# UtkuKaradeniz/scrabble-gan

Measured on AMD Instinct MI355X. Metric: train-step images/sec @ 32×160 bs128, 1/2/4/8 GPU; % of HBM/MFMA roofline, higher is better.
Workload: dtype f32

## Files before the change

scrabble_gan_amd/csrc/conv_bf16v2.hip:

```cpp
#include "sg_conv2.h"
#include <stdlib.h>
#include <type_traits>

typedef float f32x16 __attribute__((ext_vector_type(16)));
typedef __bf16 bf16x8 __attribute__((ext_vector_type(8)));
typedef short s16x8 __attribute__((ext_vector_type(8)));
__device__ __attribute__((aligned(256))) unsigned int sg2_zero_page[64];

__device__ __forceinline__ int sg2_xcd_remap(int orig, int nwg) {
  const int q = nwg >> 3, r = nwg & 7, xcd = orig & 7;
  const int base = xcd < r ? xcd * (q + 1) : r * (q + 1) + (xcd - r) * q;
  return base + (orig >> 3);
}

__global__ __launch_bounds__(256) void k_cvt_bf16(const float* __restrict__ x, u16* __restrict__ out, long n8, int relu,
                                                  const float* __restrict__ rowscale, long rowlen) {
  for (long e = (long)blockIdx.x * blockDim.x + threadIdx.x; e < n8; e += (long)gridDim.x * blockDim.x) {
    float4 v0 = reinterpret_cast<const float4*>(x)[2 * e], v1 = reinterpret_cast<const float4*>(x)[2 * e + 1];
    if (rowscale) {
      const float s = rowscale[(8 * e) / rowlen];
      v0.x *= s; v0.y *= s; v0.z *= s; v0.w *= s; v1.x *= s; v1.y *= s; v1.z *= s; v1.w *= s;
    }
    if (relu) {
      v0.x = fmaxf(v0.x, 0.f); v0.y = fmaxf(v0.y, 0.f); v0.z = fmaxf(v0.z, 0.f); v0.w = fmaxf(v0.w, 0.f);
      v1.x = fmaxf(v1.x, 0.f); v1.y = fmaxf(v1.y, 0.f); v1.z = fmaxf(v1.z, 0.f); v1.w = fmaxf(v1.w, 0.f);
    }
    bf16x8 h;
    h[0] = (__bf16)v0.x; h[1] = (__bf16)v0.y; h[2] = (__bf16)v0.z; h[3] = (__bf16)v0.w;
    h[4] = (__bf16)v1.x; h[5] = (__bf16)v1.y; h[6] = (__bf16)v1.z; h[7] = (__bf16)v1.w;
    reinterpret_cast<bf16x8*>(out)[e] = h;
  }
}

extern "C" int sg_cvt_bf16(const float* x, void* out, long n, int relu, const float* rowscale, long rowlen, void* stream) {
  if (!x || !out || n < 0 || (n & 7) || (rowscale && (rowlen <= 0 || (rowlen & 7)))) return SG_ERR_ARG;
  if (n == 0) return SG_OK;
  SG_KERNEL(k_cvt_bf16, dim3(sg_grid_for(n / 8, 256)), dim3(256), 0, (hipStream_t)stream, x, (u16*)out, n / 8, relu, rowscale, rowlen);
  return sg_launch_status();
}

__global__ __launch_bounds__(256) void k_cvt_bf16_bias(const float* __restrict__ x, u16* __restrict__ out, u16* __restrict__ out_plain, long M,
                                                       int C, const float* __restrict__ rowscale, long rows_per_sample,
                                                       float* __restrict__ dbias, int rows_per_block) {
  __shared__ float red[256 * 8];
  const int c8 = C >> 3;
  int CL = 256;
  while (CL > c8) CL >>= 1;
  const int RL = 256 / CL;
  const int cl = threadIdx.x % CL, rl = threadIdx.x / CL;
  const long m0 = (long)blockIdx.x * rows_per_block;
  const long m1 = m0 + rows_per_block < M ? m0 + rows_per_block : M;
  for (int cg0 = 0; cg0 < c8; cg0 += CL) {
    const int cg = cg0 + cl;
    float s[8] = {0.f, 0.f, 0.f, 0.f, 0.f, 0.f, 0.f, 0.f};
    if (cg < c8) {
      for (long m = m0 + rl; m < m1; m += RL) {
        const float4* src = reinterpret_cast<const float4*>(x + m * C + 8 * cg);
        float4 v0 = src[0], v1 = src[1];
        if (out_plain) {
          bf16x8 hp;
          hp[0] = (__bf16)v0.x; hp[1] = (__bf16)v0.y; hp[2] = (__bf16)v0.z; hp[3] = (__bf16)v0.w;
          hp[4] = (__bf16)v1.x; hp[5] = (__bf16)v1.y; hp[6] = (__bf16)v1.z; hp[7] = (__bf16)v1.w;
          *reinterpret_cast<bf16x8*>(out_plain + m * C + 8 * cg) = hp;
        }
        if (rowscale) {
          const float f = rowscale[m / rows_per_sample];
          v0.x *= f; v0.y *= f; v0.z *= f; v0.w *= f; v1.x *= f; v1.y *= f; v1.z *= f; v1.w *= f;
        }
        bf16x8 hh;
        hh[0] = (__bf16)v0.x; hh[1] = (__bf16)v0.y; hh[2] = (__bf16)v0.z; hh[3] = (__bf16)v0.w;
        hh[4] = (__bf16)v1.x; hh[5] = (__bf16)v1.y; hh[6] = (__bf16)v1.z; hh[7] = (__bf16)v1.w;
        *reinterpret_cast<bf16x8*>(out + m * C + 8 * cg) = hh;
        s[0] += v0.x; s[1] += v0.y; s[2] += v0.z; s[3] += v0.w; s[4] += v1.x; s[5] += v1.y; s[6] += v1.z; s[7] += v1.w;
      }
    }
    if (RL > 1) {
#pragma unroll
      for (int j = 0; j < 8; ++j) red[j * 256 + threadIdx.x] = s[j];
      __syncthreads();
      for (int st = RL >> 1; st > 0; st >>= 1) {
        if (rl < st) {
#pragma unroll
          for (int j = 0; j < 8; ++j) red[j * 256 + threadIdx.x] += red[j * 256 + threadIdx.x + st * CL];
        }
        __syncthreads();
      }
#pragma unroll
      for (int j = 0; j < 8; ++j) s[j] = red[j * 256 + threadIdx.x];
      __syncthreads();
    }
    if (rl == 0 && cg < c8) {
#pragma unroll
      for (int j = 0; j < 8; ++j) atomicAdd(dbias + 8 * cg + j, s[j]);
    }
  }
}

extern "C" int sg_cvt_bf16_bias(const float* x, void* out, void* out_plain, long M, int C, const float* rowscale, long rows_per_sample,
                                float* dbias, void* stream) {
  if (!x || !out || !dbias || M < 0 || C <= 0 || (C & 7) || (rowscale && rows_per_sample <= 0)) return SG_ERR_ARG;
  if (M == 0) return SG_OK;
  long r = (M + 1023) / 1024;
  if (sg_deterministic()) r = M;
  const int rpb = (int)(r < 32 ? 32 : r);
  SG_KERNEL(k_cvt_bf16_bias, dim3((unsigned)((M + rpb - 1) / rpb)), dim3(256), 0, (hipStream_t)stream, x, (u16*)out, (u16*)out_plain, M, C,
                     rowscale, rows_per_sample, dbias, rpb);
  return sg_launch_status();
}

constexpr int SG2_BM = 256, SG2_BK = 64;
constexpr int SG2_TILE = SG2_BM * SG2_BK * 2;
constexpr int SG2_LDS = 4 * SG2_TILE;

template <int BN, int ES, bool RELU, int BMT = 256, int NWO = 0>
__global__ __launch_bounds__((NWO ? NWO : (BMT == 256 ? 8 : 4)) * 64, 2) void sg_igemm_bf16v2_kernel(const SgIgemm2Args p) {
  extern __shared__ __attribute__((aligned(1024))) unsigned char smem[];
  constexpr int BM = BMT, BK = 128 / ES;
  constexpr int NW = NWO ? NWO : (BM == 256 ? 8 : 4);
  constexpr int ATILE = BM * 128;
  constexpr int WN = BN / 64, WM = NW / WN;
  constexpr int TM = BM / WM / 32, TN = 2;
  constexpr int BQ = BN / (8 * NW);
  constexpr int AQ = BM / (8 * NW);
  static_assert(BM == 256 || (BM == 128 && (BN == 128 || (BN == 64 && ES == 4))), "tile configurations");
  static_assert(NWO == 0 || (NWO == 8 && BM == 128 && ES == 4), "eight waves: the fp32 128 x 128 tile only");
  constexpr int BTILE = BN * 128;
  const int tid = threadIdx.x;
  const int lane = tid & 63;
  const int wave = __builtin_amdgcn_readfirstlane(tid >> 6);
  const int wm = wave / WN, wn = wave % WN;

  const int M = p.Bn * p.Hg * p.Wg;
  const int HW = p.Hg * p.Wg;
  const int n_tiles = p.N / BN;
  int wg, split, nsplit;
  int bid = (int)blockIdx.x;
  if constexpr (ES == 4 && BMT == 128) bid += p.block0;
  if (bid < p.full_tiles) {
    wg = sg2_xcd_remap(bid, p.full_tiles);
    split = 0;
    nsplit = 1;
  } else {
    const int tail_tiles = p.n_tiles_total - p.full_tiles;
    const int u = sg2_xcd_remap(bid - p.full_tiles, tail_tiles * p.tail_split);
    nsplit = p.tail_split;
    split = u / tail_tiles;
    wg = p.full_tiles + (u - split * tail_tiles);
  }
  const int m0 = (wg / n_tiles) * BM;
  const int n0 = (wg % n_tiles) * BN;
  const int grp = p.group_rows ? m0 / p.group_rows : 0;
  const int grp_row0 = grp * p.group_rows;
  const int kchunks = p.Ca / BK;
  const int KT_all = p.ntaps * kchunks;
  const int kt_begin = (int)(((long)KT_all * split) / nsplit);
  const int KT = (int)(((long)KT_all * (split + 1)) / nsplit) - kt_begin;

  const int lrow = lane >> 3, lslot = lane & 7;
  const unsigned char* zero = reinterpret_cast<const unsigned char*>(sg2_zero_page) + 16 * lslot;
  unsigned a_off[4], a_msk[4], b_off[4];
#pragma unroll
  for (int i = 0; i < 4; ++i) {
    const int r = (NW * i + wave) * 8 + lrow;
    const int chunk = lslot ^ ((r >> 1) & 7);
    const int m = m0 + r;
    const bool ok = m < M;
// ... 1389 lines not shown
```

scrabble_gan_amd/csrc/conv_winograd.hip:

```cpp
#include "sg_conv2.h"
#include "wino_f43.h"
#include <stdlib.h>

#define WINO_F 16

static inline long wino_tp(long T) { return (T + 127) / 128 * 128; }


__global__ __launch_bounds__(256) void k_wino_filter(const float* __restrict__ in, float* __restrict__ U, long NK, int flip) {
  for (long e = (long)blockIdx.x * 256 + threadIdx.x; e < NK; e += (long)gridDim.x * 256) {
    float g[3][3];
#pragma unroll
    for (int a = 0; a < 3; ++a)
#pragma unroll
      for (int b = 0; b < 3; ++b) g[a][b] = in[(size_t)((flip ? 2 - a : a) * 3 + (flip ? 2 - b : b)) * NK + e];
    float h[4][3];
#pragma unroll
    for (int b = 0; b < 3; ++b) {
      h[0][b] = g[0][b];
      h[1][b] = 0.5f * (g[0][b] + g[1][b] + g[2][b]);
      h[2][b] = 0.5f * (g[0][b] - g[1][b] + g[2][b]);
      h[3][b] = g[2][b];
    }
#pragma unroll
// ... 438 lines not shown
  return (long)sizeof(float) * wino_planes(tile) * wino_tp(wino_tiles(B, H, W, tile)) * ((long)Cin + Cout);
}

extern "C" int sg_wino_filter(const float* w_nk, float* u, int N, int K, int flip, int tile, void* stream) {
  if (!w_nk || !u || N <= 0 || K <= 0 || (tile != 2 && tile != 4)) return SG_ERR_ARG;
  const long NK = (long)N * K;
  if (tile == 2) SG_KERNEL(k_wino_filter, dim3(sg_grid_for(NK, 256)), dim3(256), 0, (hipStream_t)stream, w_nk, u, NK, flip);
  else SG_KERNEL(k_w43_filter, dim3(sg_grid_for(NK, 256)), dim3(256), 0, (hipStream_t)stream, w_nk, u, NK, flip);
  return sg_launch_status();
}

static int wino_input_impl(const float* x, float* V, int B, int H, int W, int C, int relu, int tile, int ups, void* stream);
extern "C" int sg_wino_input(const float* x, float* V, int B, int H, int W, int C, int relu, int tile, void* stream) {
  return wino_input_impl(x, V, B, H, W, C, relu, tile, 0, stream);
}
extern "C" int sg_wino_input_ups(const float* x_half, float* V, int B, int H, int W, int C, int tile, void* stream) {
  if (tile != 4) return SG_ERR_UNSUPPORTED;
  return wino_input_impl(x_half, V, B, H, W, C, 0, tile, 1, stream);
}
static int wino_input_impl(const float* x, float* V, int B, int H, int W, int C, int relu, int tile, int ups, void* stream) {
  if (!x || !V) return SG_ERR_ARG;
  if (!wino_shape_ok(B, H, W, C, 64, tile)) return SG_ERR_UNSUPPORTED;
  if (ups) {
    const long Tu = wino_tiles(B, H, W, 4);
    SG_KERNEL((k_w43_in<false, v4f, true>), dim3(sg_grid_for(Tu * (C / 4), 256)), dim3(256), 0, (hipStream_t)stream, x, V, H, W, C, Tu, wino_tp(Tu));
    return sg_launch_status();
  }
  const long T = wino_tiles(B, H, W, tile), Tp = wino_tp(T);
  hipStream_t s = (hipStream_t)stream;
  const dim3 grid(sg_grid_for(T * (C / 4), 256)), block(256);
  if (tile == 2) {
    if (relu) SG_KERNEL(k_wino_in<true>, grid, block, 0, s, x, V, H, W, C, T, Tp);
    else SG_KERNEL(k_wino_in<false>, grid, block, 0, s, x, V, H, W, C, T, Tp);
  } else {
    if (wino_vec() == 2) {
      const dim3 grid2(sg_grid_for(T * (C / 2), 256));
      if (relu) SG_KERNEL((k_w43_in<true, v2f>), grid2, block, 0, s, x, V, H, W, C, T, Tp);
      else SG_KERNEL((k_w43_in<false, v2f>), grid2, block, 0, s, x, V, H, W, C, T, Tp);
    } else {
      if (relu) SG_KERNEL((k_w43_in<true, v4f>), grid, block, 0, s, x, V, H, W, C, T, Tp);
      else SG_KERNEL((k_w43_in<false, v4f>), grid, block, 0, s, x, V, H, W, C, T, Tp);
    }
  }
  return sg_launch_status();
}

extern "C" int sg_wino_gemm(const float* V, const float* u, float* Mt, int B, int H, int W, int K, int N, int tile, void* stream) {
  if (!V || !u || !Mt) return SG_ERR_ARG;
  if (!wino_shape_ok(B, H, W, K, N, tile)) return SG_ERR_UNSUPPORTED;
  const long Tp = wino_tp(wino_tiles(B, H, W, tile));
  const int F = wino_planes(tile);
  if (F * Tp >= (1L << 31) - 256) return SG_ERR_UNSUPPORTED;
  SgIgemm2Args g{};
  g.a = reinterpret_cast<const u16*>(V);
  g.w = reinterpret_cast<const u16*>(u);
  g.out = Mt;
  g.Bn = (int)(F * Tp); g.Ha = 1; g.Wa = 1; g.Ca = K; g.Hg = 1; g.Wg = 1; g.a_sy = 1; g.a_sx = 1;
  g.Ho = 1; g.Wo = 1; g.N = N; g.o_sy = 1; g.o_sx = 1; g.o_oy = 0; g.o_ox = 0;
  g.ntaps = 1; g.flags = 0;
  g.taps[0] = SgTap{0, 0, 0};
  g.group_rows = (int)Tp;
  g.a_group_bytes = (long)sizeof(float) * Tp * K;
  g.w_group_bytes = (long)sizeof(float) * N * K;
  return sg_launch_igemm_bf16v2(g, (hipStream_t)stream, nullptr, 4);
}

extern "C" int sg_wino_output(const float* Mt, float* y, const float* bias, const float* bias2, const float* mask, int B, int H, int W, int N,
                              int flags, int tile, void* stream) {
  if (!Mt || !y) return SG_ERR_ARG;
  if (!wino_shape_ok(B, H, W, 32, N, tile) || (flags & (SG_TANH_OUT | SG_RELU_IN))) return SG_ERR_UNSUPPORTED;
  if ((flags & SG_POOL2_OUT) && (tile != 4 || mask || (flags & SG_RELU_OUT))) return SG_ERR_UNSUPPORTED;
  const long T = wino_tiles(B, H, W, tile), Tp = wino_tp(T);
  const dim3 grid(sg_grid_for(T * (N / 4), 256)), block(256);
  if (flags & SG_POOL2_OUT) {
    SG_KERNEL((k_w43_out<v4f, true>), grid, block, 0, (hipStream_t)stream, Mt, y, bias, bias2, mask, H, W, N, T, Tp, flags);
    return sg_launch_status();
  }
  if (tile == 2) SG_KERNEL(k_wino_out, grid, block, 0, (hipStream_t)stream, Mt, y, bias, bias2, mask, H, W, N, T, Tp, flags);
  else if (wino_vec() == 2) SG_KERNEL(k_w43_out<v2f>, dim3(sg_grid_for(T * (N / 2), 256)), block, 0, (hipStream_t)stream, Mt, y, bias, bias2, mask, H, W, N, T, Tp, flags);
  else SG_KERNEL(k_w43_out<v4f>, grid, block, 0, (hipStream_t)stream, Mt, y, bias, bias2, mask, H, W, N, T, Tp, flags);
  return sg_launch_status();
}

static int wino_conv(const float* a, const float* u, const float* bias, const float* bias2, const float* mask, float* out, int B, int H, int W,
                     int K, int N, int flags, int tile, void* workspace, long workspace_bytes, hipStream_t s) {
  if (!a || !u || !out || !workspace) return SG_ERR_ARG;
  if (!wino_shape_ok(B, H, W, K, N, tile) || (flags & SG_TANH_OUT)) return SG_ERR_UNSUPPORTED;
  if (workspace_bytes < sg_wino_workspace_bytes(B, H, W, K, N, tile)) return SG_ERR_ARG;
  const long Tp = wino_tp(wino_tiles(B, H, W, tile));
  float* V = reinterpret_cast<float*>(workspace);
  float* Mt = V + (size_t)wino_planes(tile) * Tp * K;
  int rc = wino_input_impl(a, V, B, H, W, K, (flags & SG_RELU_IN) != 0, tile, (flags & SG_UPS2_IN) != 0, s);
  if (rc != SG_OK) return rc;
  rc = sg_wino_gemm(V, u, Mt, B, H, W, K, N, tile, s);
  if (rc != SG_OK) return rc;
  return sg_wino_output(Mt, out, bias, bias2, mask, B, H, W, N, flags & ~(SG_RELU_IN | SG_UPS2_IN), tile, s);
}

extern "C" int sg_conv2d_fwd_wino(const float* x, const float* u_fwd, const float* bias, const float* bias2, float* y, int B, int H, int W,
                                  int Cin, int Cout, int flags, int tile, void* workspace, long workspace_bytes, void* stream) {
  return wino_conv(x, u_fwd, bias, bias2, nullptr, y, B, H, W, Cin, Cout, flags, tile, workspace, workspace_bytes, (hipStream_t)stream);
}

extern "C" int sg_conv2d_bwd_data_wino(const float* dy, const float* u_bwd, const float* mask, float* dx, int B, int H, int W, int Cin,
                                       int Cout, int flags, int tile, void* workspace, long workspace_bytes, void* stream) {
  if (flags & (SG_RELU_IN | SG_RELU_OUT | SG_POOL2_OUT)) return SG_ERR_ARG;
  if ((flags & SG_UPS2_IN) && tile != 4) return SG_ERR_UNSUPPORTED;
  return wino_conv(dy, u_bwd, nullptr, nullptr, mask, dx, B, H, W, Cout, Cin, flags, tile, workspace, workspace_bytes, (hipStream_t)stream);
}

extern "C" long sg_wino_wgrad_workspace_bytes(int B, int H, int W, int Cin, int Cout, int tile) {
  if (!wino_geom_ok(B, H, W, tile) || Cin <= 0 || Cout <= 0) return 0;
  const long Tp = wino_tp(wino_tiles(B, H, W, tile));
  return (long)sizeof(float) * (wino_planes(tile) * (Tp * ((long)Cin + Cout) + (long)Cin * Cout) + (long)WINO_DB_PARTS * Cout);
}

static int wino_grad_input_impl(const float* dy, float* Qt, const float* sample_scale, float* db, float* db_scratch, int B, int H, int W,
                                int N, int tile, int ups, void* stream);
extern "C" int sg_wino_grad_input(const float* dy, float* Qt, const float* sample_scale, float* db, float* db_scratch, int B, int H, int W,
                                  int N, int tile, void* stream) {
  return wino_grad_input_impl(dy, Qt, sample_scale, db, db_scratch, B, H, W, N, tile, 0, stream);
}
extern "C" int sg_wino_grad_input_ups(const float* dy_half, float* Qt, const float* sample_scale, float* db, float* db_scratch, int B, int H,
                                      int W, int N, int tile, void* stream) {
  if (tile != 4) return SG_ERR_UNSUPPORTED;
  return wino_grad_input_impl(dy_half, Qt, sample_scale, db, db_scratch, B, H, W, N, tile, 1, stream);
}
static int wino_grad_input_impl(const float* dy, float* Qt, const float* sample_scale, float* db, float* db_scratch, int B, int H, int W,
                                int N, int tile, int ups, void* stream) {
  if (!dy || !Qt) return SG_ERR_ARG;
  if (!wino_geom_ok(B, H, W, tile) || (N & 3) || N <= 0) return SG_ERR_UNSUPPORTED;
  const long T = wino_tiles(B, H, W, tile), Tp = wino_tp(T);
  hipStream_t s = (hipStream_t)stream;
  const dim3 grid(sg_grid_for(T * (N / 4), 256)), block(256);
  float* part = db ? db_scratch : nullptr;
  if (part && hipMemsetAsync(part, 0, sizeof(float) * (size_t)WINO_DB_PARTS * N, s) != hipSuccess) return SG_ERR_LAUNCH;
  if (ups) SG_KERNEL((k_w43_dy<v4f, true>), grid, block, 0, s, dy, Qt, sample_scale, db, part, H, W, N, T, Tp);
  else if (tile == 2) SG_KERNEL(k_wino_dy, grid, block, 0, s, dy, Qt, sample_scale, db, part, H, W, N, T, Tp);
  else if (wino_vec() == 2) SG_KERNEL(k_w43_dy<v2f>, dim3(sg_grid_for(T * (N / 2), 256)), block, 0, s, dy, Qt, sample_scale, db, part, H, W, N, T, Tp);
  else SG_KERNEL(k_w43_dy<v4f>, grid, block, 0, s, dy, Qt, sample_scale, db, part, H, W, N, T, Tp);
  if (part) SG_KERNEL(k_wino_db_finish, dim3(sg_cdiv(N, 256)), dim3(256), 0, s, part, db, N);
  return sg_launch_status();
}

extern "C" int sg_wino_wgrad_gemm(const float* V, const float* Qt, float* dU, int B, int H, int W, int K, int N, int tile, long v_plane_rows,
                                  void* stream) {
  if (!V || !Qt || !dU) return SG_ERR_ARG;
  if (!wino_geom_ok(B, H, W, tile) || (K & 3) || (N & 3) || K <= 0 || N <= 0) return SG_ERR_UNSUPPORTED;
  const long T = wino_tiles(B, H, W, tile), Tp = wino_tp(T);
  if (v_plane_rows != 0 && v_plane_rows < T) return SG_ERR_ARG;
  if (T >= (1L << 31) - 256) return SG_ERR_UNSUPPORTED;
  const int F = wino_planes(tile);
  hipStream_t s = (hipStream_t)stream;
  if (hipMemsetAsync(dU, 0, sizeof(float) * (size_t)F * K * N, s) != hipSuccess) return SG_ERR_LAUNCH;
  SgWgradArgs a{};
  a.p = V; a.q = Qt; a.dw = dU;
  a.Bn = (int)T; a.Hp = 1; a.Wp = 1; a.Cp = K; a.p_sy = 1; a.p_sx = 1;
  a.Hq = 1; a.Wq = 1; a.Cq = N; a.q_sy = 1; a.q_sx = 1; a.Hg = 1; a.Wg = 1;
  a.ntaps = F; a.flags = 0;
  a.p_plane = (v_plane_rows ? v_plane_rows : Tp) * K;
  a.q_plane = Tp * N;
  return sg_launch_wgrad(a, s);
}

extern "C" int sg_wino_filter_grad(const float* dU, float* dw, int K, int N, int tile, void* stream) {
  if (!dU || !dw || K <= 0 || N <= 0 || (tile != 2 && tile != 4)) return SG_ERR_ARG;
  const long KN = (long)K * N;
  if (tile == 2) SG_KERNEL(k_wino_dw, dim3(sg_grid_for(KN, 256)), dim3(256), 0, (hipStream_t)stream, dU, dw, KN);
  else SG_KERNEL(k_w43_dw, dim3(sg_grid_for(KN, 256)), dim3(256), 0, (hipStream_t)stream, dU, dw, KN);
  return sg_launch_status();
}

extern "C" int sg_conv2d_bwd_weight_wino(const float* x, const float* dy, float* dw, float* db, const float* sample_scale, int B, int H, int W,
                                         int Cin, int Cout, int flags, int tile, void* workspace, long workspace_bytes, void* stream) {
  if (!x || !dy || !dw || !workspace) return SG_ERR_ARG;
  if (!wino_shape_ok(B, H, W, Cin, 64, tile) || (Cout & 3)) return SG_ERR_UNSUPPORTED;
  if (workspace_bytes < sg_wino_wgrad_workspace_bytes(B, H, W, Cin, Cout, tile)) return SG_ERR_ARG;
  const long Tp = wino_tp(wino_tiles(B, H, W, tile));
  const int F = wino_planes(tile);
  float* V = reinterpret_cast<float*>(workspace);
  float* Qt = V + (size_t)F * Tp * Cin;
  float* dU = Qt + (size_t)F * Tp * Cout;
  int rc = sg_wino_input(x, V, B, H, W, Cin, (flags & SG_RELU_IN) != 0, tile, stream);
  if (rc != SG_OK) return rc;
  if ((flags & SG_UPS2_IN) && tile != 4) return SG_ERR_UNSUPPORTED;
  rc = wino_grad_input_impl(dy, Qt, sample_scale, db, dU + (size_t)F * Cin * Cout, B, H, W, Cout, tile, (flags & SG_UPS2_IN) != 0, stream);
  if (rc != SG_OK) return rc;
  rc = sg_wino_wgrad_gemm(V, Qt, dU, B, H, W, Cin, Cout, tile, 0, stream);
  if (rc != SG_OK) return rc;
  return sg_wino_filter_grad(dU, dw, Cin, Cout, tile, stream);
}
```

scrabble_gan_amd/csrc/sg_conv2.h:

```cpp
#pragma once
#include "sg_conv.h"

typedef unsigned short u16;

#define SG2_IDENT_OUT 32

struct SgIgemm2Args {
  const u16* a;
  const u16* w;
  float* out;
  u16* out16;
  const float* bias;
  const float* bias2;
  const float* mask;
  const u16* mask16;
  const float* amax_a;
  const float* amax_w;
  float* amax_out;
  const float* amax_rowscale;
  int Bn, Ha, Wa, Ca;
  int Hg, Wg, a_sy, a_sx;
  int Ho, Wo, N, o_sy, o_sx, o_oy, o_ox;
  int ntaps, flags;
  int full_tiles, tail_split, n_tiles_total;
  int group_rows;
  long a_group_bytes, w_group_bytes;
  SgTap taps[SG_MAX_TAPS];
  int block0;
};

int sg_launch_igemm_bf16v2(const SgIgemm2Args& a_in, hipStream_t s, long* twin_rows_done, int es);
```

scrabble_gan_amd/ops.py:

```python
from __future__ import annotations

import os as _os
from typing import Optional, Tuple

import torch

from . import operands as _operands
from ._lib import call, lib

RELU_IN, ACCUM, RELU_OUT, TANH_OUT = 1, 2, 4, 8
MMA_BF16 = 256
BN_EPS = 1e-3


class KernelTimer:

    def __init__(self, only=None):
        self.records = {}
        self.shapes = {}
        self.nbytes = {}
        self.only = only
        self.roof = {}

    def wants(self, family):
# ... 435 lines not shown
    elif kind == "t_bwd":
        call("sg_pack_filter_bf16", _p(w), out.data_ptr(), kh * kw, w.shape[2], w.shape[3], 1, _stream())
    elif kind == "fwd":
        call("sg_pack_filter_bf16", _p(w), out.data_ptr(), kh * kw, Cin, Cout, 1, _stream())
    else:
        call("sg_pack_filter_bf16", _p(w), out.data_ptr(), kh * kw, Cout, Cin, 0, _stream())
    _PACK_CACHE[key] = (w, out)
    return out


def _bf16_ok(K: int, N: int) -> bool:
    return _low() and K % 8 == 0 and N > 32 and K > 1


USE_V2 = _os.environ.get("SG_BF16_V2", "1") == "1"


def _amax_slot(like: torch.Tensor) -> torch.Tensor:
    return _OPERANDS.amax_slot(_stream(), like.device)


def _want_amax() -> bool:
    return CONV_DTYPE == "fp8" and not _FP8_BLOCK[0]


_amax_put = _OPERANDS.put_amax
_amax_get = _OPERANDS.get_amax


def _result_copies(out: torch.Tensor, want16, amax: bool):
    t16 = torch.empty(out.shape, device=out.device, dtype=torch.bfloat16) if want16 else None
    return t16, (_amax_slot(out) if amax else None)


def _result_register(out: torch.Tensor, t16, am, scale) -> None:
    if am is not None:
        _amax_put(out, am, scale)
    if t16 is not None:
        _twin_put(out, t16)


def new_step() -> None:
    _OPERANDS.new_step(WINO_KEEP_V)


def end_step() -> None:
    _OPERANDS.end_step()


_touch = _OPERANDS.touch


def bf16_scaled(t: torch.Tensor, rowscale: torch.Tensor) -> torch.Tensor:
    e = _OPERANDS.get_grad_bf16(t, rowscale)
    if e is None:
        e = _OPERANDS.put_grad_bf16(t, rowscale, cvt_bf16(t, rowscale=rowscale), None)
    return e.data


_twin_put = _OPERANDS.put_bf16
_twin_get = _OPERANDS.get_bf16


def cvt_bf16(t: torch.Tensor, relu=False, rowscale=None) -> torch.Tensor:
    _chk(t, rowscale)
    out = torch.empty(t.shape, device=t.device, dtype=torch.bfloat16)
    n = t.numel()
    assert n % 8 == 0
    with _hbm("cvt_bf16", t, out):
        call("sg_cvt_bf16", _p(t), out.data_ptr(), n, int(relu), _p(rowscale), (n // rowscale.numel()) if rowscale is not None else 8, _stream())
    return out


def cvt_bf16_bias(t: torch.Tensor, rowscale, db: torch.Tensor, want_plain: bool = False):
    _chk(t, rowscale, db)
    out = torch.empty(t.shape, device=t.device, dtype=torch.bfloat16)
    plain = torch.empty(t.shape, device=t.device, dtype=torch.bfloat16) if want_plain else None
    C = t.shape[-1]
    M = t.numel() // C
    with _hbm("cvt_bf16", t, out, plain):
        call("sg_cvt_bf16_bias", _p(t), out.data_ptr(), None if plain is None else plain.data_ptr(), M, C, _p(rowscale),
             (M // rowscale.numel()) if rowscale is not None else 1, _p(db), _stream())
    return (out, plain) if want_plain else out


def grad_operand(dy: torch.Tensor, sample_scale, want_colsum: bool):
    e = _OPERANDS.get_grad_bf16(dy, sample_scale)
    plain = _twin_get(dy)
    if e is None or (want_colsum and e.colsum is None):
        colsum = torch.zeros(dy.shape[-1], device=dy.device, dtype=torch.float32)
        if sample_scale is None:
            t16 = cvt_bf16_bias(dy, None, colsum)
            if plain is None:
                _twin_put(dy, t16)
        elif plain is None and _operands.whole(dy):
            t16, p16 = cvt_bf16_bias(dy, sample_scale, colsum, want_plain=True)
            _twin_put(dy, p16)
        else:
            t16 = cvt_bf16_bias(dy, sample_scale, colsum)
        e = _OPERANDS.put_grad_bf16(dy, sample_scale, t16, colsum)
    return e.data, e.colsum


def bf16_of(t: torch.Tensor) -> torch.Tensor:
    t16 = _twin_get(t)
    if t16 is None:
        t16 = cvt_bf16(t)
        _twin_put(t, t16)
    return t16


USE_F32_V2 = _os.environ.get("SG_F32_V2", "1") == "1"


F32_V2_MIN_TILES = 512


def _f32v2_ok(K: int, N: int, kh: int, kw: int, same: bool, pixels: int) -> bool:
    if not (USE_F32_V2 and CONV_DTYPE == "f32" and K % 32 == 0 and N % 64 == 0 and (same or (kh == 1 and kw == 1))):
        return False
    tiles = -(-pixels // 256) * -(-N // 256)
    return tiles >= F32_V2_MIN_TILES and (F32_V2_MIN_TILES == 0 or kh * kw * K >= 1024)


USE_WINOGRAD = _os.environ.get("SG_WINOGRAD", "1") == "1"
WINO_TILE = int(_os.environ.get("SG_WINO_TILE", "4"))
WINO_MIN_C = {2: int(_os.environ.get("SG_WINO_MIN_C", "128")), 4: int(_os.environ.get("SG_WINO4_MIN_C", "64"))}
WINO_MIN_KN = {2: int(_os.environ.get("SG_WINO_MIN_KN", "32768")), 4: int(_os.environ.get("SG_WINO4_MIN_KN", "16384"))}
WINO4_WGRAD_MIN_TILES = 128
_WINO_WS = {}
WINO_KEEP_V = _os.environ.get("SG_WINO_KEEP_V", "1") == "1"


def _wino_v_get(x: torch.Tensor, relu_in: bool, tile: int):
    hit = _OPERANDS.kept(x, relu_in, tile)
    if hit is None:
        return None
    e, t0 = hit
    if e.stream != _stream():
        e.V.record_stream(torch.cuda.current_stream())
    return e.V.data_ptr() + 4 * t0 * x.shape[3], e.plane_rows


def _wino_tile(H: int, W: int) -> int:
    return 4 if (WINO_TILE == 4 and H % 4 == 0 and W % 4 == 0) else 2


WINO_ROW_GAIN = float(_os.environ.get("SG_WINO_ROW_GAIN", "0.75"))
WINO_N_MULT = int(_os.environ.get("SG_WINO_N_MULT", "64"))


def set_wino_persist(mode: int, wgs: int = 0) -> None:
    lib().sg_debug_set_wino_persist(int(mode), int(wgs))


def _wino_rows_ok(B, H: int, W: int, tile: int) -> bool:
    if B is None or WINO_ROW_GAIN <= 0 or DETERMINISTIC:
        return True
    T = B * (H // tile) * (W // tile)
    return (tile + 2) ** 2 * (-(-T // 128) * 128) <= WINO_ROW_GAIN * 9 * (-(-(B * H * W) // 128) * 128)


def _wino_ok(K: int, N: int, kh: int, kw: int, same: bool, H: int, W: int, B=None) -> bool:
    if not (USE_WINOGRAD and CONV_DTYPE == "f32" and kh == 3 and kw == 3 and same and H % 2 == 0 and W % 2 == 0 and K % 32 == 0 and N % WINO_N_MULT == 0):
        return False
    t = _wino_tile(H, W)
    return min(K, N) >= WINO_MIN_C[t] and K * N >= WINO_MIN_KN[t] and _wino_rows_ok(B, H, W, t)


def _wino_workspace(nbytes: int, like: torch.Tensor) -> torch.Tensor:
    key = _stream()
    buf = _WINO_WS.get(key)
    if buf is None or buf.numel() < nbytes:
        _WINO_WS.pop(key, None)
        buf = None
        buf = torch.empty(nbytes, device=like.device, dtype=torch.uint8)
        _WINO_WS[key] = buf
    return buf


def _wino_conv(a, w, out, bias, bias2, mask, K: int, N: int, relu_in: bool, flags: int, tag, ups: bool = False) -> None:
    B, H, W, _ = a.shape
    if ups:
        H, W = 2 * H, 2 * W
        flags |= UPS2_IN
    tile = _wino_tile(H, W)
    P = (tile + 2) ** 2
    fwd = tag[0] == "wino_fwd"
    u = packed_filter(w, ("wino_fwd%d" if fwd else "wino_bwd%d") % tile)
    T = B * (H // tile) * (W // tile)
    Tp = -(-T // 128) * 128
    nbytes = 4 * P * Tp * (K + N)
    s = _stream()
    keep = (fwd and _OPERANDS.keeping and a.storage_offset() == 0 and _wino_wgrad_ok(K, N, 3, 3, True, H, W)
            and (tile == 2 or T >= WINO4_WGRAD_MIN_TILES))
    if keep:
        Vt = torch.empty(P * Tp * K, device=a.device, dtype=torch.float32)
        _OPERANDS.keep(a, relu_in, tile, Vt, Tp, s)
        V = Vt.data_ptr()
        Mt = _wino_workspace(4 * P * Tp * N, a).data_ptr()
        if PROFILER is None:
            call("sg_wino_input", _p(a), V, B, H, W, K, int(relu_in), tile, s)
            call("sg_wino_gemm", V, _p(u), Mt, B, H, W, K, N, tile, s)
            call("sg_wino_output", Mt, _p(out), _p(bias), _p(bias2), None, B, H, W, N, flags, tile, s)
            return
    else:
        ws = _wino_workspace(nbytes, a)
        V = ws.data_ptr()
        Mt = V + 4 * P * Tp * K
    if PROFILER is None:
        if fwd:
            call("sg_conv2d_fwd_wino", _p(a), _p(u), _p(bias), _p(bias2), _p(out), B, H, W, K, N, flags | (1 if relu_in else 0), tile, V, nbytes, s)
        else:
            call("sg_conv2d_bwd_data_wino", _p(a), _p(u), _p(mask), _p(out), B, H, W, N, K, flags, tile, V, nbytes, s)
        return
    with _hbm("wino_transform", a, flops=0.0) as _:
        if PROFILER is not None and PROFILER.wants("wino_transform"):
            PROFILER.nbytes["wino_transform"] = PROFILER.nbytes.get("wino_transform", 0.0) + 4.0 * P * T * K
        if ups:
            call("sg_wino_input_ups", _p(a), V, B, H, W, K, tile, s)
        else:
            call("sg_wino_input", _p(a), V, B, H, W, K, int(relu_in), tile, s)
    with _timed("igemm_wino", 2.0 * P * Tp * K * N, False, tag):
        if PROFILER is not None and PROFILER.wants("igemm_wino"):
            PROFILER.nbytes["igemm_wino"] = PROFILER.nbytes.get("igemm_wino", 0.0) + 4.0 * P * (Tp * K + N * K + Tp * N)
        call("sg_wino_gemm", V, _p(u), Mt, B, H, W, K, N, tile, s)
    with _hbm("wino_transform", out, mask, flops=0.0):
        if PROFILER is not None and PROFILER.wants("wino_transform"):
            PROFILER.nbytes["wino_transform"] = PROFILER.nbytes.get("wino_transform", 0.0) + 4.0 * P * T * N
        call("sg_wino_output", Mt, _p(out), _p(bias), _p(bias2), _p(mask), B, H, W, N, flags & ~UPS2_IN, tile, s)


def _wino_wgrad_ok(Cin: int, Cout: int, kh: int, kw: int, same: bool, H: int, W: int) -> bool:
    if not (USE_WINOGRAD and CONV_DTYPE == "f32" and not DETERMINISTIC and kh == 3 and kw == 3 and same and H % 2 == 0 and W % 2 == 0
            and Cin % 32 == 0 and Cout % 64 == 0):
        return False
    t = _wino_tile(H, W)
    return min(Cin, Cout) >= WINO_MIN_C[t] and Cin * Cout >= (min(WINO_MIN_KN[4], 4096) if t == 4 else WINO_MIN_KN[2])


def _wino_wgrad(x, dy, dw, db, sample_scale, relu_in: bool, ups: bool = False) -> None:
    B, H, W, Cin = x.shape
    Cout = dy.shape[3]
    tile = _wino_tile(H, W)
    if tile == 4 and B * (H // 4) * (W // 4) < WINO4_WGRAD_MIN_TILES:
        tile = 2
    assert not ups or tile == 4
    P = (tile + 2) ** 2
    T = B * (H // tile) * (W // tile)
    Tp = -(-T // 128) * 128
    nbytes = 4 * (P * (Tp * (Cin + Cout) + Cin * Cout) + 64 * Cout)
    ws = _wino_workspace(nbytes, x)
    V = ws.data_ptr()
    Qt = V + 4 * P * Tp * Cin
    dU = Qt + 4 * P * Tp * Cout
    s = _stream()
    kept = _wino_v_get(x, bool(relu_in), tile)
    v_rows = 0
    if kept is not None:
        V, v_rows = kept
    elif PROFILER is None:
        call("sg_conv2d_bwd_weight_wino", _p(x), _p(dy), _p(dw), _p(db), _p(sample_scale), B, H, W, Cin, Cout, (1 if relu_in else 0) | (UPS2_IN if ups else 0),
             tile, V, nbytes, s)
        return
    with _hbm("wino_transform", x if kept is None else None, dy):
        if PROFILER is not None and PROFILER.wants("wino_transform"):
            PROFILER.nbytes["wino_transform"] = PROFILER.nbytes.get("wino_transform", 0.0) + 4.0 * P * T * ((Cin if kept is None else 0) + Cout)
        if kept is None:
            call("sg_wino_input", _p(x), V, B, H, W, Cin, int(relu_in), tile, s)
        call("sg_wino_grad_input_ups" if ups else "sg_wino_grad_input", _p(dy), Qt, _p(sample_scale), _p(db), dU + 4 * P * Cin * Cout, B, H, W, Cout, tile, s)
    with _timed("wgrad_wino", 2.0 * P * T * Cin * Cout, False, ("wino_wgrad", B, H, W, Cin, Cout, 3)):
        if PROFILER is not None and PROFILER.wants("wgrad_wino"):
            PROFILER.nbytes["wgrad_wino"] = PROFILER.nbytes.get("wgrad_wino", 0.0) + 4.0 * P * (T * (Cin + Cout) + Cin * Cout)
        call("sg_wino_wgrad_gemm", V, Qt, dU, B, H, W, Cin, Cout, tile, v_rows, s)
    with _hbm("wino_transform", dw, dw):
        if PROFILER is not None and PROFILER.wants("wino_transform"):
            PROFILER.nbytes["wino_transform"] = PROFILER.nbytes.get("wino_transform", 0.0) + 4.0 * P * Cin * Cout
        call("sg_wino_filter_grad", dU, _p(dw), Cin, Cout, tile, s)


def _v2_ok(K: int, N: int, kh: int, kw: int, same: bool) -> bool:
    return USE_V2 and _low() and K % 64 == 0 and N % 64 == 0 and (same or (kh == 1 and kw == 1))


POOL2_OUT, UPS2_IN = 16, 64
FUSE_POOL = _os.environ.get("SG_FUSE_POOL", "1") == "1"


def conv2d_avgpool_fwd(x, w, bias=None, relu_in=False):
    _chk(x, w, bias)
    B, H, W, Cin = x.shape
    kh, kw, wc, Cout = w.shape
    if FUSE_POOL and _wino_ok(Cin, Cout, kh, kw, True, H, W, B) and _wino_tile(H, W) == 4:
        out = empty(B, H // 2, W // 2, Cout, like=x)
        _wino_conv(x, w, out, bias, None, None, Cin, Cout, relu_in, POOL2_OUT, ("wino_fwd", B, H, W, Cin, Cout, kh))
        return out
    return avgpool2_add_fwd(conv2d_fwd(x, w, bias, relu_in=relu_in))


def pooled_grad_foldable(B: int, H: int, W: int, Cin: int, Cout: int, want_dw: bool) -> bool:
    if not (FUSE_POOL and CONV_DTYPE == "f32"):
        return False
    if not (_wino_ok(Cout, Cin, 3, 3, True, H, W, B) and _wino_tile(H, W) == 4):
        return False
    if want_dw and not (_wino_wgrad_ok(Cin, Cout, 3, 3, True, H, W) and B * (H // 4) * (W // 4) >= WINO4_WGRAD_MIN_TILES):
        return False
# ... 870 lines not shown
```

Measured before the change: 949.3.

## Add persistent direct-to-LDS MFMA kernel for Winograd weight-gradient GEMM

Adds a persistent kernel for the Winograd filter-gradient batched GEMM. It streams V and Qt tiles straight into LDS with global_load_lds double buffering interleaved with f32 MFMA, and splits the tile (reduction) dimension into chunks that are accumulated atomically. Work items are remapped across XCDs, and the chunk count is chosen by a heuristic based on CU count. It is enabled by default for large or small-channel shapes with at least 2048 tiles, replacing the generic wgrad launcher for those shapes. In exchange it adds atomics and a memset, and makes results non-deterministic unless deterministic mode is set.

```diff
diff --git a/scrabble_gan_amd/csrc/conv_bf16v2.hip b/scrabble_gan_amd/csrc/conv_bf16v2.hip
--- a/scrabble_gan_amd/csrc/conv_bf16v2.hip
+++ b/scrabble_gan_amd/csrc/conv_bf16v2.hip
@@ -6,12 +6,6 @@
 typedef __bf16 bf16x8 __attribute__((ext_vector_type(8)));
 typedef short s16x8 __attribute__((ext_vector_type(8)));
 __device__ __attribute__((aligned(256))) unsigned int sg2_zero_page[64];
-
-__device__ __forceinline__ int sg2_xcd_remap(int orig, int nwg) {
-  const int q = nwg >> 3, r = nwg & 7, xcd = orig & 7;
-  const int base = xcd < r ? xcd * (q + 1) : r * (q + 1) + (xcd - r) * q;
-  return base + (orig >> 3);
-}
 
 __global__ __launch_bounds__(256) void k_cvt_bf16(const float* __restrict__ x, u16* __restrict__ out, long n8, int relu,
                                                   const float* __restrict__ rowscale, long rowlen) {
diff --git a/scrabble_gan_amd/csrc/conv_wino_wgrad.hip b/scrabble_gan_amd/csrc/conv_wino_wgrad.hip
--- /dev/null
+++ b/scrabble_gan_amd/csrc/conv_wino_wgrad.hip
@@ -0,0 +1,263 @@
+#include "sg_conv2.h"
+#include <stdlib.h>
+
+typedef float f32x16 __attribute__((ext_vector_type(16)));
+__device__ __attribute__((aligned(256))) unsigned int sgww_zero_page[64];
+
+struct SgWinoWgradArgs {
+  const float* v;
+  const float* q;
+  float* du;
+  long v_plane, q_plane;
+  int T, K, N, F;
+  int mchunk, nchunks;
+  int c_tiles, n_tiles, items;
+  int atomic;
+};
+
+template <int OFF>
+__device__ __forceinline__ void sgww_dsr(float& d, unsigned addr) {
+  asm volatile("ds_read_b32 %0, %1 offset:%2" : "=v"(d) : "v"(addr), "n"(OFF));
+}
+
+template <int NW>
+__global__ __launch_bounds__(NW * 64, 2) void sg_wino_wgrad_persist_kernel(const SgWinoWgradArgs p) {
+  static_assert(NW == 4, "four waves of 64 x 64");
+  extern __shared__ __attribute__((aligned(1024))) unsigned char smem[];
+  typedef unsigned long long u64;
+  constexpr int BK = 32, ATILE = BK * 512, STAGE = 2 * ATILE;
+  const int tid = threadIdx.x;
+  const int lane = tid & 63;
+  const int wave = __builtin_amdgcn_readfirstlane(tid >> 6);
+  const int wm = wave >> 1, wn = wave & 1;
+  const int grid = (int)gridDim.x;
+  const int K = p.K, N = p.N, T = p.T, items = p.items;
+
+  struct Item { int f, c0, n0, m_begin, m_end; };
+  auto decode = [&](int vb) {
+    const int it = sg2_xcd_remap(vb, items);
+    Item r;
+    int x = it / p.n_tiles;
+    r.n0 = (it - x * p.n_tiles) * 128;
+    int y = x / p.c_tiles;
+    r.c0 = (x - y * p.c_tiles) * 128;
+    const int chunk = y / p.F;
+    r.f = y - chunk * p.F;
+    r.m_begin = chunk * p.mchunk;
+    r.m_end = min(T, r.m_begin + p.mchunk);
+    return r;
+  };
+
+  const int lrow = 2 * wave + (lane >> 5), lcol = 4 * (lane & 31);
+  const u64 zsrc = (u64)reinterpret_cast<uintptr_t>(sgww_zero_page) + 16u * (unsigned)(lane & 15);
+  const unsigned qstride_a = 4u * 8u * (unsigned)K, qstride_b = 4u * 8u * (unsigned)N;
+  int lvb = (int)blockIdx.x, lk = 0, l_kt = 0, l_rows = 0;
+  u64 a_src = 0, b_src = 0;
+  bool a_cok = false, b_cok = false, l_live = false;
+  auto cursor_item = [&]() {
+    l_live = lvb < items;
+    if (!l_live) return;
+    const Item it = decode(lvb);
+    l_rows = it.m_end - it.m_begin;
+    l_kt = (l_rows + BK - 1) / BK;
+    a_cok = it.c0 + lcol < K;
+    b_cok = it.n0 + lcol < N;
+    a_src = (u64)reinterpret_cast<uintptr_t>(p.v) + 4ull * ((u64)it.f * (u64)p.v_plane + (u64)(it.m_begin + lrow) * (u64)K + (u64)(it.c0 + lcol));
+    b_src = (u64)reinterpret_cast<uintptr_t>(p.q) + 4ull * ((u64)it.f * (u64)p.q_plane + (u64)(it.m_begin + lrow) * (u64)N + (u64)(it.n0 + lcol));
+  };
+  auto advance = [&]() {
+    if (!l_live) return;
+    ++lk;
+    l_rows -= BK;
+    a_src += 4ull * BK * (u64)K;
+    b_src += 4ull * BK * (u64)N;
+    if (lk >= l_kt) {
+      lk = 0;
+      lvb += grid;
+      cursor_item();
+    }
+  };
+  auto issue_part = [&](int st, int q) {
+    if (!l_live) return;
+    const bool rok = lrow + 8 * q < l_rows;
+    const u64 sa = (rok && a_cok) ? a_src + (u64)((unsigned)q * qstride_a) : zsrc;
+    const u64 sb = (rok && b_cok) ? b_src + (u64)((unsigned)q * qstride_b) : zsrc;
+    unsigned char* dst_a = smem + st * STAGE + (NW * q + wave) * 1024;
+    unsigned char* dst_b = dst_a + ATILE;
+    __builtin_amdgcn_global_load_lds((const __attribute__((address_space(1))) void*)(uintptr_t)sa, (__attribute__((address_space(3))) void*)dst_a, 16, 0, 0);
+    __builtin_amdgcn_global_load_lds((const __attribute__((address_space(1))) void*)(uintptr_t)sb, (__attribute__((address_space(3))) void*)dst_b, 16, 0, 0);
+  };
+
+  f32x16 acc[2][2];
+  const int frow = lane & 31, khalf = lane >> 5;
+  const unsigned lds0 = (unsigned)(uintptr_t)(__attribute__((address_space(3))) unsigned char*)smem;
+  const unsigned a_rd = lds0 + 512u * (unsigned)khalf + 4u * (unsigned)(wm * 64 + frow);
+  const unsigned b_rd = lds0 + (unsigned)ATILE + 512u * (unsigned)khalf + 4u * (unsigned)(wn * 64 + frow);
+  float af[2][2], bf[2][2];
+#define SGWW_READ_FRAGS(aa, bb, s, slot)                                                     \
+  do {                                                                                       \
+    sgww_dsr<(s) * 1024>(af[slot][0], aa);                                                   \
+    sgww_dsr<(s) * 1024 + 128>(af[slot][1], aa);                                             \
+    sgww_dsr<(s) * 1024>(bf[slot][0], bb);                                                   \
+    sgww_dsr<(s) * 1024 + 128>(bf[slot][1], bb);                                             \
+  } while (0)
+  auto mma = [&](int slot) {
+#pragma unroll
+    for (int i = 0; i < 2; ++i)
+#pragma unroll
+      for (int j = 0; j < 2; ++j) acc[i][j] = __builtin_amdgcn_mfma_f32_32x32x2f32(af[slot][i], bf[slot][j], acc[i][j], 0, 0, 0);
+  };
+  auto mma_dma = [&](int slot, int st) {
+#pragma unroll
+    for (int i = 0; i < 2; ++i)
+#pragma unroll
+      for (int j = 0; j < 2; ++j) {
+        acc[i][j] = __builtin_amdgcn_mfma_f32_32x32x2f32(af[slot][i], bf[slot][j], acc[i][j], 0, 0, 0);
+        __builtin_amdgcn_sched_barrier(0);
+        issue_part(st, 2 * i + j);
+        __builtin_amdgcn_sched_barrier(0);
+      }
+    advance();
+  };
+#define SGWW_STEP(aa, bb, s_next, slot_next, slot_cur)                                       \
+  do {                                                                                       \
+    SGWW_READ_FRAGS(aa, bb, s_next, slot_next);                                              \
+    asm volatile("s_waitcnt lgkmcnt(4)" ::: "memory");                                       \
+    __builtin_amdgcn_sched_barrier(0);                                                       \
+    mma(slot_cur);                                                                           \
+    __builtin_amdgcn_sched_barrier(0);                                                       \
+  } while (0)
+  auto k_tile = [&](int st) {
+    const unsigned aa = a_rd + (unsigned)(st * STAGE), bb = b_rd + (unsigned)(st * STAGE);
+    const unsigned an = a_rd + (unsigned)((st ^ 1) * STAGE), bn = b_rd + (unsigned)((st ^ 1) * STAGE);
+    SGWW_STEP(aa, bb, 1, 1, 0);
+    SGWW_STEP(aa, bb, 2, 0, 1);
+    SGWW_STEP(aa, bb, 3, 1, 0);
+    SGWW_STEP(aa, bb, 4, 0, 1);
+    SGWW_STEP(aa, bb, 5, 1, 0);
+    SGWW_STEP(aa, bb, 6, 0, 1);
+    SGWW_STEP(aa, bb, 7, 1, 0);
+    SGWW_STEP(aa, bb, 8, 0, 1);
+    SGWW_STEP(aa, bb, 9, 1, 0);
+    SGWW_STEP(aa, bb, 10, 0, 1);
+    SGWW_STEP(aa, bb, 11, 1, 0);
+    SGWW_STEP(aa, bb, 12, 0, 1);
+    SGWW_STEP(aa, bb, 13, 1, 0);
+    SGWW_STEP(aa, bb, 14, 0, 1);
+    SGWW_STEP(aa, bb, 15, 1, 0);
+    asm volatile("s_waitcnt vmcnt(0) lgkmcnt(0)" ::: "memory");
+    __builtin_amdgcn_s_barrier();
+    SGWW_READ_FRAGS(an, bn, 0, 0);
+    __builtin_amdgcn_sched_barrier(0);
+    mma_dma(1, st);
+    __builtin_amdgcn_sched_barrier(0);
+  };
+
+  cursor_item();
+  {
+#pragma unroll
+    for (int q = 0; q < 4; ++q) issue_part(0, q);
+    advance();
+    asm volatile("s_waitcnt vmcnt(0)" ::: "memory");
+    __builtin_amdgcn_s_barrier();
+#pragma unroll
+    for (int q = 0; q < 4; ++q) issue_part(1, q);
+    advance();
+    SGWW_READ_FRAGS(a_rd, b_rd, 0, 0);
+    __builtin_amdgcn_sched_barrier(0);
+  }
+  int st = 0;
+  for (int cvb = (int)blockIdx.x; cvb < items; cvb += grid) {
+    const Item it = decode(cvb);
+    const int KT = (it.m_end - it.m_begin + BK - 1) / BK;
+#pragma unroll
+    for (int i = 0; i < 2; ++i)
+#pragma unroll
+      for (int j = 0; j < 2; ++j)
+#pragma unroll
+        for (int r = 0; r < 16; ++r) acc[i][j][r] = 0.f;
+    for (int kt = 0; kt < KT; ++kt) {
+      k_tile(st);
+      st ^= 1;
+    }
+    float* du = p.du + ((size_t)it.f * (size_t)K + (size_t)(it.c0 + wm * 64)) * (size_t)N + (size_t)(it.n0 + wn * 64 + frow);
+    const int c_left = K - (it.c0 + wm * 64), n_left = N - (it.n0 + wn * 64 + frow);
+    const bool whole = it.c0 + 128 <= K && it.n0 + 128 <= N;
+#pragma unroll
+    for (int i = 0; i < 2; ++i)
+#pragma unroll
+      for (int j = 0; j < 2; ++j)
+#pragma unroll
+        for (int r = 0; r < 16; ++r) {
+          const int row = 32 * i + (r & 3) + 8 * (r >> 2) + 4 * khalf;
+          if (!whole && (row >= c_left || 32 * j >= n_left)) continue;
+          float* d = du + (size_t)row * (size_t)N + 32 * j;
+          if (p.atomic) atomicAdd(d, acc[i][j][r]);
+          else *d = acc[i][j][r];
+        }
+    __builtin_amdgcn_sched_barrier(0);
+  }
+  asm volatile("s_waitcnt lgkmcnt(0)" ::: "memory");
+}
+
+static int gww_mode = getenv("SG_WINO_WGRAD_DMA") ? atoi(getenv("SG_WINO_WGRAD_DMA")) : 1;
+static int gww_wgs = getenv("SG_WINO_WGRAD_DMA_WGS") ? atoi(getenv("SG_WINO_WGRAD_DMA_WGS")) : 0;
+extern "C" void sg_debug_set_wino_wgrad_dma(int mode, int wgs) {
+  gww_mode = mode;
+  gww_wgs = wgs;
+}
+
+bool sg_wino_wgrad_dma_wanted(long T, int K, int N) {
+  if (gww_mode <= 0) return false;
+  if (K <= 64 || N <= 64 || (K & 3) || (N & 3)) return false;
+  if (gww_mode >= 2) return true;
+  return T >= 2048 && ((K >= 512 && N >= 512) || (K <= 128 && N <= 128));
+}
+
+int sg_launch_wino_wgrad_dma(const float* V, const float* Qt, float* dU, long T, int K, int N, int F, long v_plane, long q_plane, hipStream_t s) {
+  static bool attr_done = false;
+  static int cus = 0;
+  if (!attr_done) {
+    int dev = 0;
+    if (hipGetDevice(&dev) != hipSuccess || hipDeviceGetAttribute(&cus, hipDeviceAttributeMultiprocessorCount, dev) != hipSuccess || cus <= 0) cus = 256;
+    if (hipFuncSetAttribute(reinterpret_cast<const void*>(sg_wino_wgrad_persist_kernel<4>), hipFuncAttributeMaxDynamicSharedMemorySize, 65536) != hipSuccess) {
+      (void)hipGetLastError();
+      return SG_ERR_UNSUPPORTED;
+    }
+    attr_done = true;
+  }
+  const int c_tiles = sg_cdiv(K, 128), n_tiles = sg_cdiv(N, 128);
+  const long combos = (long)F * c_tiles * n_tiles;
+  if (combos <= 0 || T <= 0) return SG_OK;
+  const long max_chunks = (T + 255) / 256;
+  long nchunks = 1;
+  double best = 1e30;
+  for (long c = (6 * cus + combos - 1) / combos; c <= (12 * cus + combos - 1) / combos; ++c) {
+    const long cc = c < 1 ? 1 : (c > max_chunks ? max_chunks : c);
+    const long W = combos * cc;
+    const long per_cu = (W + cus - 1) / cus;
+    const double occ_pen = (per_cu % 2) ? 1.01 : 1.0;
+    const double loss = (double)per_cu * cus / (double)W * (1.0 + 0.002 * cc) * occ_pen;
+    if (loss < best) {
+      best = loss;
+      nchunks = cc;
+    }
+  }
+  if (sg_deterministic()) nchunks = 1;
+  long mchunk = (T + nchunks - 1) / nchunks;
+  mchunk = (mchunk + 31) / 32 * 32;
+  nchunks = (T + mchunk - 1) / mchunk;
+  if (combos * nchunks >= (1L << 31) - 1) return SG_ERR_UNSUPPORTED;
+  SgWinoWgradArgs a{};
+  a.v = V; a.q = Qt; a.du = dU;
+  a.v_plane = v_plane; a.q_plane = q_plane;
+  a.T = (int)T; a.K = K; a.N = N; a.F = F;
+  a.mchunk = (int)mchunk; a.nchunks = (int)nchunks;
+  a.c_tiles = c_tiles; a.n_tiles = n_tiles; a.items = (int)(combos * nchunks);
+  a.atomic = nchunks > 1;
+  if (a.atomic && hipMemsetAsync(dU, 0, sizeof(float) * (size_t)F * K * N, s) != hipSuccess) return SG_ERR_LAUNCH;
+  int grid = a.items < 2 * cus ? a.items : 2 * cus;
+  if (gww_wgs > 0 && grid > gww_wgs) grid = gww_wgs;
+  SG_KERNEL((sg_wino_wgrad_persist_kernel<4>), dim3(grid), dim3(256), 65536, s, a);
+  return sg_launch_status();
+}
diff --git a/scrabble_gan_amd/csrc/conv_winograd.hip b/scrabble_gan_amd/csrc/conv_winograd.hip
--- a/scrabble_gan_amd/csrc/conv_winograd.hip
+++ b/scrabble_gan_amd/csrc/conv_winograd.hip
@@ -614,6 +614,7 @@
   if (T >= (1L << 31) - 256) return SG_ERR_UNSUPPORTED;
   const int F = wino_planes(tile);
   hipStream_t s = (hipStream_t)stream;
+  if (sg_wino_wgrad_dma_wanted(T, K, N)) return sg_launch_wino_wgrad_dma(V, Qt, dU, T, K, N, F, (v_plane_rows ? v_plane_rows : Tp) * K, Tp * N, s);
   if (hipMemsetAsync(dU, 0, sizeof(float) * (size_t)F * K * N, s) != hipSuccess) return SG_ERR_LAUNCH;
   SgWgradArgs a{};
   a.p = V; a.q = Qt; a.dw = dU;
diff --git a/scrabble_gan_amd/csrc/sg_conv2.h b/scrabble_gan_amd/csrc/sg_conv2.h
--- a/scrabble_gan_amd/csrc/sg_conv2.h
+++ b/scrabble_gan_amd/csrc/sg_conv2.h
@@ -30,3 +30,12 @@
 };
 
 int sg_launch_igemm_bf16v2(const SgIgemm2Args& a_in, hipStream_t s, long* twin_rows_done, int es);
+
+__device__ __forceinline__ int sg2_xcd_remap(int orig, int nwg) {
+  const int q = nwg >> 3, r = nwg & 7, xcd = orig & 7;
+  const int base = xcd < r ? xcd * (q + 1) : r * (q + 1) + (xcd - r) * q;
+  return base + (orig >> 3);
+}
+
+bool sg_wino_wgrad_dma_wanted(long T, int K, int N);
+int sg_launch_wino_wgrad_dma(const float* V, const float* Qt, float* dU, long T, int K, int N, int F, long v_plane, long q_plane, hipStream_t s);
diff --git a/scrabble_gan_amd/ops.py b/scrabble_gan_amd/ops.py
--- a/scrabble_gan_amd/ops.py
+++ b/scrabble_gan_amd/ops.py
@@ -611,6 +611,10 @@
 
 def set_wino_persist(mode: int, wgs: int = 0) -> None:
     lib().sg_debug_set_wino_persist(int(mode), int(wgs))
+
+
+def set_wino_wgrad_dma(mode: int, wgs: int = 0) -> None:
+    lib().sg_debug_set_wino_wgrad_dma(int(mode), int(wgs))
 
 
 def _wino_rows_ok(B, H: int, W: int, tile: int) -> bool:
```

Measured after the change: 954.3, median of 6. Within noise of the previous version (+0.5%).
